# warmshao/ChatTTSPlus

Hardware: AMD Instinct MI355X
Metric: decode tokens/s (higher is better)
Workload: dtype f32

## Files before the change

chatttsplus_amd/csrc/gpt_engine.hip:

```cpp
#include <fcntl.h>
#include <stdarg.h>
#include <stdio.h>
#include <stdlib.h>
#include <string.h>
#include <sys/file.h>
#include <sys/stat.h>
#include <unistd.h>

#include <cmath>
#include <map>
#include <mutex>
#include <string>
#include <atomic>
#include <thread>
#include <vector>

#include "../../include/ctts_hip.h"
#include "kernels.h"
#include "persist.h"
#include "roctx_range.h"

static thread_local char g_err[512] = "";
void ctts_set_error(const char* fmt, ...) {
    va_list ap;
// ... 44 lines not shown
    float* logits_text = nullptr;
    float* lnf = nullptr;
    float* emb_code = nullptr;
    float* emb_text = nullptr;
    int vocab_text = 0;
    int vocab_text_head = 0;
    float* rope = nullptr;
    float *rope_pre = nullptr, *rope_dec = nullptr;
    int rope_n = 0;
    char* kv = nullptr;
    size_t kv_bytes = 0;
    float* sk_scratch = nullptr; size_t sk_cap_floats = 0;
    float *x_dec = nullptr, *x_last = nullptr, *x_pre = nullptr, *q_buf = nullptr, *part_ml = nullptr, *part_o = nullptr, *logits = nullptr;
    void* act = nullptr;
    void* attn_packed = nullptr;
    void* norm_packed = nullptr;
    int split_rows = 4;
    float* dpart = nullptr;
    int launched = 0;
    int nbg2_rows = 33;
    int force_splits = 0;
    int down_sk_rows = 9;
    float* sk_slab = nullptr; int* sk_cnt = nullptr;
    int opt_gen = 0;
    int graph_gen = 0;
    int valu_rows = 2;
    int persist_rows = 0;
    bool persist_ok = false;
    char* pimg = nullptr;
    char* pimg_head = nullptr;
    int persist_delay_u = -1;
    int prefill_pp_blocks = 1;
    int prefill_small_blocks = 192;
    int prefill_ring4_blocks = 256;
    int prefill_sk_rows = 2048;
    int attn_wide_blocks = 0;
    int persist_share_keys = 384;
    int persist_lora = 1;
    int persist_heads = 1;
    unsigned long long* pl_g = nullptr;
    unsigned* pl_epoch = nullptr;
    int* pl_error = nullptr;
    unsigned long long* pl_ts = nullptr;
    int pl_ts_on = 0;
    int persist_fault = 0;
    int persist_pair_keys = 704;
// ... 212 lines not shown
    {"persistent_share_keys", &ctts_gpt::persist_share_keys, 64, 384, OPT_MAX, OPT_MAX, OPT_RW, 0, HOOK_NONE},
    {"persistent_lora", &ctts_gpt::persist_lora, OPT_ANY, OPT_RW | OPT_FLAG, 0, HOOK_NONE},
    {"persistent_heads", &ctts_gpt::persist_heads, OPT_ANY, OPT_RW | OPT_FLAG, 0, HOOK_NONE},
    {"persistent_layers_per_launch", &ctts_gpt::persist_lpl, OPT_MIN(0), OPT_RW, 0, HOOK_NONE},
    {"persistent_schedule", &ctts_gpt::persist_sched, 1, 1, 3, 1, OPT_RW, 0, HOOK_NONE},
    {"lora_fold", &ctts_gpt::lora_fold, 0, 1, 3, 1, OPT_RW, 0, HOOK_NONE},
    {"persistent_fault", &ctts_gpt::persist_fault, OPT_MIN(0), OPT_RW, 0, HOOK_NONE},
    {"persistent_pair_keys", &ctts_gpt::persist_pair_keys, OPT_MIN(0), OPT_RW, 0, HOOK_NONE},
    {"persistent_max_keys", &ctts_gpt::persist_max_keys, OPT_MIN(0), OPT_RW, 0, HOOK_NONE},
    {"persistent_splits", &ctts_gpt::persist_splits, OPT_RANGE(0, PL_SMAX), OPT_RW, 0, HOOK_NONE},
    {"persistent_pace", &ctts_gpt::persist_pace, 0, -1, 64, 64, OPT_RW, 0, HOOK_NONE},
    {"persistent_delay_att", &ctts_gpt::persist_delay_att, OPT_RANGE(0, 256), OPT_RW, 0, HOOK_NONE},
    {"persistent_delay", &ctts_gpt::persist_delay, OPT_RANGE(0, 256), OPT_RW, 0, HOOK_NONE},
    {"persistent_delay_act", &ctts_gpt::persist_delay_act, OPT_RANGE(0, 256), OPT_RW, 0, HOOK_NONE},
    {"persistent_delay_x", &ctts_gpt::persist_delay_x, OPT_RANGE(0, 256), OPT_RW, 0, HOOK_NONE},
    {"persistent_nap_qkv", &ctts_gpt::persist_nap_qkv, OPT_RANGE(0, 256), OPT_RW, 0, HOOK_NONE},
    {"persistent_nap", &ctts_gpt::persist_nap, OPT_RANGE(0, 256), OPT_RW, 0, HOOK_NONE},
    {"persistent_poll", &ctts_gpt::persist_poll, OPT_ANY, OPT_RW, 0, HOOK_POLL},
    {"persistent_timestamps", &ctts_gpt::pl_ts_on, OPT_ANY, OPT_RW | OPT_FLAG, 0, HOOK_TIMESTAMPS},
    {"decode_splits", &ctts_gpt::force_splits, OPT_ANY, OPT_RW | OPT_PIN, 1, HOOK_DECODE_SPLITS},
    {"split_rows", &ctts_gpt::split_rows, OPT_RANGE(0, 32), OPT_RW | OPT_PIN, 0, HOOK_NONE},
    {"nbg2_rows", &ctts_gpt::nbg2_rows, OPT_MIN(17), OPT_RW | OPT_PIN, 0, HOOK_NONE},
    {"down_splitk_rows", &ctts_gpt::down_sk_rows, OPT_MIN(0), OPT_RW | OPT_PIN, 1, HOOK_NONE},
    {"graph_steps", &ctts_gpt::graph_steps, OPT_RANGE(1, 64), OPT_RW, 0, HOOK_NONE},
    {"graph_steps_persistent", &ctts_gpt::graph_steps_persist, OPT_RANGE(1, 64), OPT_RW, 0, HOOK_NONE},
    {"text_rows_live", &ctts_gpt::text_live, OPT_ANY, OPT_R, 0, HOOK_NONE},
    {"lora_mlp_live", &ctts_gpt::lora_mlp, OPT_ANY, OPT_R, 0, HOOK_NONE},
};
static const OptRow* find_option(const char* name, int access) {
    for (const OptRow& o : g_options) if (!strcmp(name, o.name)) return (o.flags & access) ? &o : nullptr;
    return nullptr;
}

extern "C" int ctts_gpt_get_option(ctts_gpt* h, const char* name, int* value) {
    if (!h || !name || !value) { ctts_set_error("get_option: null argument"); return 1; }
    const OptRow* o = find_option(name, OPT_R);
    if (!o) { ctts_set_error("get_option: unknown option '%s'", name); return 1; }
    if (h->batch_inv && (o->flags & OPT_PIN)) *value = o->pin;
    else if (o->hook == HOOK_PERSIST_ROWS) *value = (h->persist_ok || !h->finalized) ? h->persist_rows : 0;
    else *value = h->*o->field;
    return 0;
}

extern "C" int ctts_gpt_set_option(ctts_gpt* h, const char* name, int value) {
    if (!h || !name) { ctts_set_error("set_option: null argument"); return 1; }
    const OptRow* o = find_option(name, OPT_W);
// ... 507 lines not shown
    {
        long cap = (long)MB * h->cfg.max_seq;
        cap = (cap + 255) / 256 * 256;
        h->pass_rows = (int)(cap < PASS_ROWS_MAX ? cap : PASS_ROWS_MAX);
        if (const char* pr = getenv("CTTS_PASS_ROWS")) { const int v = atoi(pr); if (v >= 256 && v < h->pass_rows) h->pass_rows = v / 256 * 256; }
    }
    const int PASS_ROWS = h->pass_rows;
    const size_t act_bytes = (size_t)((PASS_ROWS + PASS_PAD) / 16) * (h->I / (h->esz == 2 ? 32 : 16)) * 1024;
    if (dev_alloc(h, (void**)&h->x_dec, (size_t)CTTS_MAX_B * H * 4) || dev_alloc(h, (void**)&h->x_last, (size_t)CTTS_MAX_B * H * 4) ||
        dev_alloc(h, (void**)&h->x_pre, (size_t)PASS_ROWS * H * 4) ||
        dev_alloc(h, (void**)&h->q_buf, (size_t)PASS_ROWS * H * 4) ||
        dev_alloc(h, (void**)&h->part_ml, (size_t)(CTTS_MAX_B + 32) * NH * SMAX * 2 * 4) ||
        dev_alloc(h, (void**)&h->part_o, (size_t)(CTTS_MAX_B + 32) * NH * SMAX * CTTS_HEAD_DIM * 4) ||
        dev_alloc(h, (void**)&h->logits, (size_t)CTTS_MAX_B * (h->NVQ * h->V > h->vocab_text_head ? h->NVQ * h->V : h->vocab_text_head) * 4) || dev_alloc(h, &h->act, act_bytes) || dev_alloc(h, (void**)&h->rope_pre, (size_t)MB * h->cfg.max_seq * 64 * 4) ||
        dev_alloc(h, (void**)&h->rope_dec, (size_t)CTTS_MAX_B * 64 * 4) || dev_alloc(h, (void**)&h->dpart, (size_t)32 * 4 * H * 4) || dev_alloc(h, &h->attn_packed, (size_t)((PASS_ROWS + PASS_PAD) / 16) * (H / (h->esz == 2 ? 32 : 16)) * 1024) ||
        dev_alloc(h, &h->norm_packed, (size_t)((PASS_ROWS + PASS_PAD) / 16) * (H / (h->esz == 2 ? 32 : 16)) * 1024) ||
        dev_alloc(h, (void**)&h->meta_pre, (size_t)MB * h->cfg.max_seq * sizeof(RowMeta)) ||
        dev_alloc(h, (void**)&h->meta_dec, CTTS_MAX_B * sizeof(RowMeta)) || dev_alloc(h, (void**)&h->meta_dec0, CTTS_MAX_B * sizeof(RowMeta)) ||
        dev_alloc(h, (void**)&h->st, sizeof(DevState)) || dev_alloc(h, (void**)&h->last_rows, CTTS_MAX_B * 4) ||
        dev_alloc(h, (void**)&h->dyn, sizeof(SamplerDyn)) || dev_alloc(h, (void**)&h->hist_ring, (size_t)CTTS_MAX_B * CTTS_NUM_VQ * 16 * 4) ||
        dev_alloc(h, (void**)&h->finend, (size_t)CTTS_MAX_B * (sizeof(RowState) + sizeof(RowSampling))) || dev_alloc(h, (void**)&h->sat, 4) ||
        dev_alloc(h, (void**)&h->cknobs, (size_t)CTTS_MAX_B * sizeof(RowSampling)) ||
        dev_alloc(h, (void**)&h->sk_slab, (size_t)(H / 16) * (CTTS_MAX_B / 16) * 4 * 256 * 4) || dev_alloc(h, (void**)&h->sk_cnt, (size_t)(H / 16) * (CTTS_MAX_B / 16) * 4) ||
        dev_alloc(h, (void**)&h->cx, (size_t)CTTS_MAX_B * H * 4) || dev_alloc(h, (void**)&h->crope, (size_t)CTTS_MAX_B * 64 * 4) ||
        dev_alloc(h, (void**)&h->cmeta, CTTS_MAX_B * sizeof(RowMeta)) || dev_alloc(h, (void**)&h->cring, (size_t)CTTS_MAX_B * CTTS_NUM_VQ * 16 * 4) ||
        dev_alloc(h, (void**)&h->cfin, (size_t)CTTS_MAX_B * sizeof(RowState)) || dev_alloc(h, (void**)&h->keep_dev, CTTS_MAX_B * 4) ||
        dev_alloc(h, &h->xh, (size_t)((CTTS_MAX_B + 32) / 16) * (H / (h->esz == 2 ? 32 : 16)) * 1024) || dev_alloc(h, (void**)&h->ssq, (size_t)(CTTS_MAX_B + 32) * (H / 16) * 4) ||
        dev_alloc(h, (void**)&h->scale_o, (size_t)(CTTS_MAX_B + 32) * 4) || dev_alloc(h, (void**)&h->scale_d, (size_t)(CTTS_MAX_B + 32) * 4) ||
        dev_alloc(h, (void**)&h->rope_dec0, (size_t)CTTS_MAX_B * 64 * 4))
        return 1;
    if (h->wsplit) {
        const size_t rows = (size_t)PASS_ROWS + PASS_PAD;
        if (dev_alloc(h, &h->sp_x_hi, rows * H * 2) || dev_alloc(h, &h->sp_x_lo, rows * H * 2) || dev_alloc(h, &h->sp_act_hi, rows * h->I * 2) || dev_alloc(h, &h->sp_act_lo, rows * h->I * 2)) return 1;
        h->sk_cap_floats = (size_t)4 * (size_t)(((PASS_ROWS < 2048 ? PASS_ROWS : 2048) + 127) / 128 * 128) * H;
        if (dev_alloc(h, (void**)&h->sk_scratch, h->sk_cap_floats * 4)) return 1;
    }
    h->knobs = (RowSampling*)(h->finend + CTTS_MAX_B);
    CTTS_HIP_CHECK(hipHostMalloc((void**)&h->host_pin, 64));
    {
        auto it = h->host.find("emb_text.weight");
        if (it != h->host.end() && it->second.size() % H == 0) {
            h->vocab_text = (int)(it->second.size() / H);
            if (dev_alloc(h, (void**)&h->emb_text, it->second.size() * 4)) return 1;
            CTTS_HIP_CHECK(hipMemcpy(h->emb_text, it->second.data(), it->second.size() * 4, hipMemcpyHostToDevice));
        }
    }
// ... 47 lines not shown
static inline int decode_splits(const ctts_gpt* h, int B, int L) {
    const int forced = tuning(h).force_splits;
    if (h->lora_rows) return 1;
    if (forced) return forced;
    int cap = 256 / (B * h->NH);
    cap = cap < 1 ? 1 : (cap > SMAX ? SMAX : cap);
    if (B <= 2) return cap;
    if (B >= 8) return 1;
    const int want = (L + 767) / 768;
    return want < 1 ? 1 : (want > cap ? cap : want);
}

struct StreamForm { bool parts, xh, logits, split; int nbg, valu; };
static inline int decode_nbg(const Tuning& t, int R, bool split) { return (R <= 16 || R < (split ? t.split_nbg2_rows : t.nbg2_rows)) ? 1 : 2; }
static StreamForm stream_form(const ctts_gpt* h, bool parts, bool xh, bool logits, bool split) {
    const Tuning t = tuning(h);
    return {parts, xh, logits, split, decode_nbg(t, h->B, split), (h->cfg.dtype == CTTS_DTYPE_F32 && h->B <= t.valu_rows) ? 1 : 0};
}
static inline StreamForm plain_form(const ctts_gpt* h) { return stream_form(h, false, false, false, false); }

struct LayerPlan {
    bool lora, lmlp;
    int S, nbg, chunks, dts, pf_kb, valu, wide_blocks, anchor, prefill_sk_rows;
    bool splitd, prepack, pfg, pfs, xhm, spd, down_sk, fuse_heads;
    int persist, per, pace, poll, delay_act, delay_u;
    StreamForm form;
};
static LayerPlan plan_layers(const ctts_gpt* h, int R, bool decode, DecodePath path) {
    LayerPlan p = {};
    const Tuning t = tuning(h);
    const int dt = h->cfg.dtype;
    p.S = path.splits; p.lora = h->lora_rows != 0; p.lmlp = p.lora && h->lora_mlp != 0;
    const bool spd_ok = decode && dt == CTTS_DTYPE_F32 && h->xh_mode && h->split_ok && h->wsplit != nullptr && !p.lora && p.S == 1 &&
                        t.split_dec_rows > 0 && R >= t.split_dec_rows && R > t.split_rows;
    p.nbg = decode ? decode_nbg(t, R, spd_ok) : (R <= 16 ? 1 : 2);
    p.chunks = (R + 16 * p.nbg - 1) / (16 * p.nbg);
    p.splitd = decode && (R <= t.split_rows) && (p.nbg == 1) && !p.lora;
    p.prepack = !decode && (p.nbg == 2) && (R > 64) && !h->no_prepack;
    p.pfg = p.prepack && (dt == CTTS_DTYPE_F16) && h->prefill_gemm_rows > 0 && (R >= h->prefill_gemm_rows) && !p.lora;
    p.pfs = (dt == CTTS_DTYPE_F32) && h->wsplit != nullptr &&
            (t.inv ? (!decode && h->split_ok) : (p.prepack && h->split_rows_min > 0 && (R >= h->split_rows_min)));
    p.xhm = decode && h->xh_mode && !p.splitd;
    p.spd = p.xhm && spd_ok;
    p.dts = p.spd ? 2 : dt;
    p.pf_kb = (p.xhm && !p.lora && (p.spd || (dt == CTTS_DTYPE_F16 && R >= 17))) ? h->prefetch_kb : 0;
    p.valu = (decode && dt == CTTS_DTYPE_F32 && R <= t.valu_rows && !p.lora) ? 1 : 0;
    p.down_sk = (p.nbg == 1 || p.spd) && R >= t.down_sk_rows && t.down_sk_rows > 0;
    p.wide_blocks = t.attn_wide_blocks; p.anchor = t.inv ? 1 : 0; p.prefill_sk_rows = t.prefill_sk_rows;
    p.form = stream_form(h, p.splitd, p.xhm, false, p.spd);
    p.persist = (decode && h->pimg != nullptr && R <= PL_MAXR) ? path.persist : 0;
    if (p.persist) {
        p.fuse_heads = h->persist_heads && R <= 2 && !h->text_mode && h->text_live == 0 && h->persist_sched == 3 && h->pimg_head != nullptr && h->dyn != nullptr;
        p.form = stream_form(h, false, false, p.fuse_heads, false);
        p.per = (h->persist_lpl > 0 && h->persist_lpl < h->L) ? h->persist_lpl : h->L;
        p.pace = h->persist_pace < 0 ? (R <= 2 ? 3 : 2) : h->persist_pace; p.poll = (h->persist_poll < 0) ? 0 : h->persist_poll;
        p.delay_act = h->persist_delay_act + 2 * (R - 1); p.delay_u = h->persist_delay_u < 0 ? 14 + 2 * R : h->persist_delay_u;
    }
    return p;
}

static int run_layers(ctts_gpt* h, float* x, const RowMeta* meta, const float* rope_rows, int R, DecodePath path, const DevState* st, hipStream_t s, StreamForm* form = nullptr) {
    const LayerPlan p = plan_layers(h, R, st != nullptr, path);
    const int dt = h->cfg.dtype, S = p.S, nbg = p.nbg, NB = 16 * nbg, chunks = p.chunks, dts = p.dts;
    const bool lora = p.lora, lmlp = p.lmlp, splitd = p.splitd, prepack = p.prepack, pfg = p.pfg, pfs = p.pfs, xhm = p.xhm, spd = p.spd;
    if (form) *form = p.form;
    if (p.persist) {
        for (int l = 0; l < h->L; l += p.per) {
            PersistArgs pa = {};
            if (p.fuse_heads && l + p.per >= h->L) {
                pa.heads = 1; pa.hw = h->pimg_head; pa.logits = h->logits; pa.n_valid = h->NVQ * h->V; pa.lnf = h->lnf; pa.dyn = h->dyn; pa.rows = h->finend;
// ... 111 lines not shown
            if (launch_gemm(dts, nbg, PRO_XH, EPI_SWIGLU, g3, chunks, s)) return 1;
        } else if (launch_gemm(dt, nbg, PRO_NORM, EPI_SWIGLU, g3, chunks, s)) return 1;
        GemmArgs g4 = a;
        g4.W = h->lw[l].d; g4.n_row_tiles = h->H / 16; g4.K = h->I; g4.xpacked = h->act; g4.x_out = x;
        if (lmlp) {
            if (pfs ? launch_lora_delta_down_split(h->sp_act_hi, h->sp_act_lo, meta, h->lora_slot_of_seq, h->lora_mA_d + mlp_l * 16 * h->I, h->lora_mB_d + mlp_l * 16 * h->H,
                                                   h->lora_mscale + mlp_l * 4, h->lora_do, R, h->H, h->I, s)
                    : launch_lora_delta_down(dt, h->act, nbg, meta, h->lora_slot_of_seq, h->lora_mA_d + mlp_l * 16 * h->I, h->lora_mB_d + mlp_l * 16 * h->H,
                                             h->lora_mscale + mlp_l * 4, h->lora_do, R, h->H, h->I, s)) return 1;
            g4.lora_delta = h->lora_do;
        }
        if (pfs) {
            if (launch_prefill_split_gemm(EPI_RESID, g4, h->lw[l].d_sp, h->sp_act_hi, h->sp_act_lo, nullptr, nullptr, sp_scale * 16.0f, sp_pol, s)) return 1;
        } else if (pfg) {
            if (launch_prefill_gemm(EPI_RESID, g4, s)) return 1;
        } else if (splitd) {
            g4.part_out = h->dpart; g4.ktiles_total = h->I / (h->esz == 2 ? 32 : 16);
            if (launch_gemm(dt, nbg, PRO_PACKED, EPI_PART, g4, chunks, s)) return 1;
        } else if (xhm) {
            g4.xh = h->xh; g4.ssq = h->ssq; g4.scale_in = h->scale_d;
            if (spd) g4.W = h->lw[l].d_sp;
            if (p.down_sk) {
                g4.ktiles_total = h->I / ((h->esz == 2 || spd) ? 32 : 16); g4.sk_slab = h->sk_slab; g4.sk_cnt = h->sk_cnt;
                if (launch_gemm(dts, nbg, PRO_PACKED, EPI_RESID_XH_SK, g4, chunks, s)) return 1;
            } else if (launch_gemm(dts, nbg, PRO_PACKED, EPI_RESID_XH, g4, chunks, s)) return 1;
        } else if (launch_gemm(dt, nbg, PRO_PACKED, EPI_RESID, g4, chunks, s)) return 1;
    }
    return 0;
}
static int run_heads(ctts_gpt* h, bool write_hidden, StreamForm form, hipStream_t s, bool mixed_text = false) {
    const int nbg = form.nbg, chunks = (h->B + 16 * nbg - 1) / (16 * nbg);
    const bool text = h->text_mode || mixed_text;
    GemmArgs a = {};
    a.st = h->st; a.R = h->B; a.eps = 1e-6f; a.meta = h->meta_dec;
    a.valu = form.valu;
    const int nv = text ? h->vocab_text_head : h->NVQ * h->V;
    a.W = text ? h->whead_text : h->whead; a.n_row_tiles = (nv + 15) / 16; a.K = h->H; a.x = h->x_dec; a.lnw = h->lnf;
    a.logits = mixed_text ? h->logits_text : h->logits; a.n_valid = nv;
    a.dyn = (write_hidden && !mixed_text) ? h->dyn : nullptr;
    a.rows = h->finend;
    a.opart = h->dpart; a.np = form.parts ? 4 : 0;
    if (form.xh && !text && h->xh_heads && (!form.split || h->whead_sp != nullptr)) {
        a.xh = h->xh; a.ssq = h->ssq; a.scale_in = h->scale_d;
        if (form.split) a.W = h->whead_sp;
        return launch_gemm(form.split ? 2 : h->cfg.dtype, nbg, PRO_XH, EPI_LOGITS, a, chunks, s);
    }
// ... 7 lines not shown
        if (!h->text_rows_on || !h->dyn_text || !h->logits_text) {
            ctts_set_error("sample / decode: a row of the batch is a text row (mode 1) but ctts_gpt_enable_text_rows has not been called for this generate state");
            return 1;
        }
        StreamForm tf = form;
        tf.logits = false;
        if (run_heads(h, false, tf, s, true)) return 1;
    }
    SamplerArgs sa = {};
    sa.dyn = h->dyn; sa.logits = h->logits; sa.V = h->text_mode ? h->vocab_text_head : h->V; sa.B = h->B; sa.st = h->st;
    sa.text_mode = h->text_mode; sa.mixed = mixed ? 1 : 0;
    sa.emb_code = h->text_mode ? h->emb_text : h->emb_code; sa.H = h->H; sa.x_next = h->x_dec; sa.meta = h->meta_dec; sa.rope = h->rope; sa.rope_rows = h->rope_dec;
    sa.hist_ring = h->hist_ring; sa.finend = h->finend;
    if (launch_sampler(sa, h->B, s)) return 1;
    if (!mixed) return 0;
    sa.dyn = h->dyn_text; sa.logits = h->logits_text; sa.V = h->vocab_text_head; sa.text_mode = 1; sa.emb_code = h->emb_text;
    return launch_sampler(sa, h->B, s);
}

static int reset_state(ctts_gpt* h, bool keep_draw, hipStream_t s) {
    h->launched = 0;
    CTTS_HIP_CHECK(hipMemsetAsync(&h->st->step, 0, 4, s));
    if (!keep_draw) CTTS_HIP_CHECK(hipMemsetAsync(&h->st->draw, 0, 4, s));
    CTTS_HIP_CHECK(hipMemsetAsync(&h->st->all_done, 0, 8, s));
    CTTS_HIP_CHECK(hipMemcpyAsync(h->meta_dec, h->meta_dec0, h->B * sizeof(RowMeta), hipMemcpyDeviceToDevice, s));
    CTTS_HIP_CHECK(hipMemsetAsync(h->io.finish, 0, h->B * 4, s));
    CTTS_HIP_CHECK(hipMemsetAsync(h->io.end_idx, 0, h->B * 4, s));
    if (!keep_draw) {
        CTTS_HIP_CHECK(hipMemcpyAsync(h->finend, h->rows_host.data(), h->B * sizeof(RowState), hipMemcpyHostToDevice, s));
    } else {
        if (launch_restart_rows(h->finend, h->B, s)) return 1;
        h->row_ctx.assign(h->B, h->T);
    }
    CTTS_HIP_CHECK(hipMemsetAsync(h->hist_ring, 0xFF, (size_t)h->B * CTTS_NUM_VQ * 16 * 4, s));
    return 0;
}

static int seat_row_adapters(ctts_gpt* h, int B, const char* who, hipStream_t s) {
    if (h->lora_slot_host.empty()) return 0;
    if (h->lora_req_host.empty()) h->lora_slot_host.assign(CTTS_MAX_B, -1);
    else h->lora_slot_host = h->lora_req_host;
    bool any = false;
    for (int b = 0; b < CTTS_MAX_B; ++b) { h->lora_row_slots[b] = (signed char)h->lora_slot_host[b]; any = any || (b < B && h->lora_slot_host[b] >= 0); }
    h->lora_rows = any ? 1 : 0;
    h->lora_mlp = 0;
    for (int b = 0; b < B; ++b) if (lora_slot_has_mlp(h, h->lora_slot_host[b])) h->lora_mlp = 1;
// ... 520 lines not shown
    (void)advance_rows(h, n_steps);
    h->launched += n_steps;
    bool persistent = false;
    for (const auto& sg : h->segs) persistent = persistent || sg.path.persist != 0;
    PersistTurnGuard turn(persistent, s);
    if (turn.rc) { ctts_set_error("decode: hipStreamWaitEvent failed"); return 1; }
    for (const auto& sg : h->segs) if (run_segment(h, sg, use_graph != 0, true, s)) return 1;
    return 0;
}

extern "C" int ctts_gpt_progress(ctts_gpt* h, int32_t* steps_done, int32_t* all_finished, void* stream) {
    if (!h) { ctts_set_error("null handle"); return 1; }
    hipStream_t s = (hipStream_t)stream;
    CTTS_HIP_CHECK(hipMemcpyAsync(h->host_pin, h->st, 16, hipMemcpyDeviceToHost, s));
    h->host_pin[12] = 0;
    if (h->pl_error) CTTS_HIP_CHECK(hipMemcpyAsync(h->host_pin + 12, h->pl_error, 4, hipMemcpyDeviceToHost, s));
    CTTS_HIP_CHECK(hipStreamSynchronize(s));
    if (steps_done) *steps_done = h->host_pin[0];
    if (all_finished) *all_finished = h->host_pin[2];
    if (h->host_pin[12] == 7) {
        ctts_set_error("per-utterance LoRA: a projection tile gave up waiting for its low-rank term (lora_worker.h); use options={'lora_fold': 0}");
        return 1;
    }
    if (h->host_pin[12] != 0) {
        ctts_set_error("persistent decode layer: a workgroup gave up waiting on edge %d (2 = q|k|v -> attention, 3 = attention -> o_proj, 4 = o_proj -> gate|up, "
                       "5 = gate|up -> down); is the GPU shared with another process?  Use options={'persistent_rows': 0}", h->host_pin[12]);
        return 1;
    }
    return 0;
}

extern "C" int ctts_gpt_progress_enqueue(ctts_gpt* h, int32_t* host_pinned4, void* stream) {
    if (!h || !host_pinned4) { ctts_set_error("progress_enqueue: null argument"); return 1; }
    CTTS_HIP_CHECK(hipMemcpyAsync(host_pinned4, h->st, 16, hipMemcpyDeviceToHost, (hipStream_t)stream));
    return 0;
}

extern "C" int ctts_gpt_saturations(ctts_gpt* h, int32_t* count, void* stream) {
    if (!h || !count || !h->sat) { ctts_set_error("saturations: bad argument"); return 1; }
    CTTS_HIP_CHECK(hipMemcpyAsync(h->host_pin + 8, h->sat, 4, hipMemcpyDeviceToHost, (hipStream_t)stream));
    CTTS_HIP_CHECK(hipStreamSynchronize((hipStream_t)stream));
    *count = h->host_pin[8];
    return 0;
}

extern "C" int ctts_gpt_rows_enqueue(ctts_gpt* h, int32_t* host_pinned_2B, void* stream) {
// ... 316 lines not shown
```

chatttsplus_amd/csrc/kernels.h:

```cpp
#pragma once
#include "common.h"

enum { PRO_NORM = 0, PRO_ATTN = 1, PRO_PACKED = 2, PRO_NORM_P = 3, PRO_XH = 4 };
enum { EPI_QKV = 0, EPI_RESID = 1, EPI_SWIGLU = 2, EPI_LOGITS = 3, EPI_RESID_P = 4, EPI_PART = 5, EPI_RESID_XH = 6, EPI_RESID_XH_SK = 7 };
#define CTTS_NPART 4

typedef unsigned long long lora_u64;
struct LoraFold {
    const float* A;
    const float* B;
    const float* scale;
    const float* lnw;
    signed char slots[CTTS_MAX_B];
    signed char ranks[32];
    lora_u64* g;
    lora_u64* g_o;
    int* err;
    int layer;
    int diag;
};

struct WPrefetch {
    const void* ptr;
    unsigned unit_bytes;
    unsigned n_units;
};

// ... 18 lines not shown
    const void* xpacked;
    float* x_out;
    float* q_out;
    void* k_cache;
    void* v_cache;
    int Lmax;
    const RowMeta* meta;
    const float* rope_rows;
    void* act_out;
    float* logits;
    int n_valid;
    void* xh;
    float* ssq;
    const float* scale_in;
    float* scale_out;
    const float* lora_delta;
    int lora_gu;
    LoraFold lf;
    int lora_w;
    int* sat;
    const RowState* rows;
    float* sk_slab;
    int* sk_cnt;
    WPrefetch pf;
    int pf_blocks;
    int valu;
};

struct AttnArgs {
    const float* q;
    const void* k_cache;
    const void* v_cache;
    int Lmax;
    int NH;
    int R;
    int S;
    const RowMeta* meta;
    const DevState* st;
    float* part_ml;
    float* part_o;
    void* packed_out;
    int nbg;
    int packed_split;
    int T, row0;
    int wide_blocks;
    int anchor;
// ... 152 lines not shown
```

chatttsplus_amd/csrc/skinny_gemm.hip:

```cpp
#include "kernels.h"
#include "lora_worker.h"

#define ATT_SMAX 8

template <typename WT> struct Mma;
template <> struct Mma<half_t> {
    __device__ static inline f32x4 run(half8 a, half8 b, f32x4 c) {
        return __builtin_amdgcn_mfma_f32_16x16x32_f16(a, b, c, 0, 0, 0);
    }
};
template <> struct Mma<float> {
    __device__ static inline f32x4 run(f32x4 a, f32x4 b, f32x4 c) {
        c = __builtin_amdgcn_mfma_f32_16x16x4f32(a[0], b[0], c, 0, 0, 0);
        c = __builtin_amdgcn_mfma_f32_16x16x4f32(a[1], b[1], c, 0, 0, 0);
        c = __builtin_amdgcn_mfma_f32_16x16x4f32(a[2], b[2], c, 0, 0, 0);
        c = __builtin_amdgcn_mfma_f32_16x16x4f32(a[3], b[3], c, 0, 0, 0);
        return c;
    }
};

struct SplitFrag { half8 hi, lo; };
template <> struct Mma<split_t> {
    __device__ static inline f32x4 run(const SplitFrag& a, const SplitFrag& b, f32x4 c) {
        c = __builtin_amdgcn_mfma_f32_16x16x32_f16(a.lo, b.hi, c, 0, 0, 0);
        c = __builtin_amdgcn_mfma_f32_16x16x32_f16(a.hi, b.lo, c, 0, 0, 0);
        c = __builtin_amdgcn_mfma_f32_16x16x32_f16(a.hi, b.hi, c, 0, 0, 0);
// ... 68 lines not shown
        const char* p = (const char*)pf.ptr + (size_t)u * pf.unit_bytes + (unsigned)(tid * 16);
        for (unsigned off = 0; off < pf.unit_bytes; off += WAVES * 1024)
            __builtin_amdgcn_global_load_lds((gptr_t)(p + off), (lptr_t)dst, 16, 0, 0);
    }
}

template <typename WT, int NBG, int WAVES, int KPW, int PRO, int EPI, int RT = 1, int VR = 0, bool LORA = false>
__global__ __launch_bounds__(WAVES * 64) void skinny_gemm_kernel(const int* done_p, const void* Wq, const void* in0, const void* in1,
                                                                  const float* resid_in, const int R, const int misc, const GemmArgs a) {
    static_assert(RT == 1 || EPI == EPI_QKV || EPI == EPI_SWIGLU, "multi-tile blocks: QKV / SwiGLU epilogues only");
    static_assert(VR == 0 || (sizeof(WT) == 4 && NBG == 1 && RT == 1 && PRO != PRO_XH && VR <= 4), "VALU products: fp32, one 16-row chunk, <= 4 rows");
    constexpr bool VALU = VR > 0;
    constexpr bool SPLIT = (WTraits<WT>::TILE_BYTES == 2048);
    typedef typename FragOf<WT>::type frag;
    constexpr int KT = WTraits<WT>::KT;
    constexpr int KTILES = WAVES * KPW;
    constexpr int K = KTILES * KT;
    constexpr int NB = 16 * NBG;
    constexpr int XS_BYTES = (PRO == PRO_PACKED || PRO == PRO_XH) ? 0 : NBG * KTILES * WTraits<WT>::TILE_BYTES;
    constexpr int PER = K / 256;
    extern __shared__ __attribute__((aligned(16))) char smem[];

    int done_v = 0;
    if (done_p != nullptr) done_v = vload_flag(done_p);
#define CTTS_EXIT_IF_DONE() if (__builtin_amdgcn_readfirstlane(done_v)) return

    const int tid = threadIdx.x, lane = tid & 63, wave = tid >> 6;
    constexpr bool PFCAP = (EPI == EPI_RESID_XH) && (PRO == PRO_PACKED) && (K == 768) && VR == 0 && !LORA;
    if constexpr (PFCAP) {
        const int xreal = (int)((unsigned)misc >> 22);
        if (__builtin_expect(xreal != 0 && (int)blockIdx.x >= xreal, 0)) {
            if (blockIdx.y == 0 && blockIdx.z == 0) {
                weight_prefetch<WAVES>(a.pf, (int)blockIdx.x - xreal, (int)gridDim.x - xreal, (int)blockIdx.x & 7, smem, tid);
            }
            return;
        }
    }
    const int chunk = blockIdx.y;
    const int row0 = chunk * NB;
    constexpr bool LORA_QKV = LORA && (EPI == EPI_QKV) && (K == 768) && (VR == 0) && (PRO == PRO_NORM || PRO == PRO_XH);
    constexpr bool LORA_O = LORA && (EPI == EPI_RESID || EPI == EPI_RESID_XH) && (K == 768) && (VR == 0) && (PRO == PRO_PACKED);
    constexpr bool LORA_GU = LORA && (EPI == EPI_SWIGLU) && (VR == 0);
    static_assert(!LORA || LORA_QKV || LORA_O || LORA_GU, "LoRA: the q/k/v and o_proj launches of a decode step (workers), the gate|up launch (epilogue term)");
    const int lw = (LORA_QKV || LORA_O) ? ((misc >> 15) & 0x7F) : 0;
    int lora_draw = 0;
#define CTTS_LORA_TAG_LO ((unsigned)a.lf.layer * 2u + (LORA_O ? 1u : 0u))
// ... 214 lines not shown
    }

    constexpr bool PREB = !VALU && (PRO == PRO_PACKED) && ((RT == 1 && NBG * KPW * (SPLIT ? 2 : 1) <= 12) || NBG * KPW * (SPLIT ? 2 : 1) <= 6);
    frag bpre[NBG][KPW];
    f32x4 bv[(VALU && PRO == PRO_PACKED) ? VR : 1][KPW];
    if (PRO == PRO_PACKED) {
        if (VALU) {
            const f32x4* xq = (const f32x4*)in0 + (size_t)chunk * NBG * kt_all * 64 + (lane & 48);
#pragma unroll
            for (int n = 0; n < VR; ++n)
#pragma unroll
                for (int i = 0; i < KPW; ++i) bv[n][i] = xq[(size_t)(kt_off + wave * KPW + i) * 64 + n];
        }
        if (PREB) {
#pragma unroll
            for (int g = 0; g < NBG; ++g)
#pragma unroll
                for (int i = 0; i < KPW; ++i) bpre[g][i] = FragIO<WT>::load(in0, (size_t)chunk * NBG * kt_all + (size_t)(g * kt_all + kt_off + wave * KPW + i), lane);
        }
        CTTS_ISSUE_WEIGHT_LOADS();
        CTTS_EXIT_IF_DONE();
    }
    float* fac_s = (float*)(smem + XS_BYTES + WAVES * NBG * 1024);
    if (PRO == PRO_XH) {
        constexpr int LPR = 64 / NB, PPL = 48 / LPR;
        f32x4 sq[PPL / 4];
        float sc_in = 1.f;
        const int n_f = lane / LPR, part = lane % LPR;
        const bool frow = (wave == WAVES - 1) && (row0 + n_f < R);
        if (frow) {
            const f32x4* sp = (const f32x4*)((const float*)in1 + (size_t)(row0 + n_f) * 48 + part * PPL);
#pragma unroll
            for (int i = 0; i < PPL / 4; ++i) sq[i] = sp[i];
            sc_in = resid_in[row0 + n_f];
        }
        {
#pragma unroll
            for (int g = 0; g < NBG; ++g)
#pragma unroll
                for (int i = 0; i < KPW; ++i) bpre[g][i] = FragIO<WT>::load(in0, (size_t)chunk * NBG * KTILES + (size_t)(g * KTILES + wave * KPW + i), lane);
        }
        CTTS_ISSUE_WEIGHT_LOADS();
        CTTS_EXIT_IF_DONE();
        if (wave == WAVES - 1) {
            float ss = 0.f;
            if (frow) {
#pragma unroll
                for (int i = 0; i < PPL / 4; ++i) ss += (sq[i][0] + sq[i][1]) + (sq[i][2] + sq[i][3]);
            }
            ss += dpp_f<DPP_XOR1>(ss);
            if (LPR == 4) ss += dpp_f<DPP_XOR2>(ss);
            if (frow && part == 0) {
                const float rs = 1.0f / sqrtf(ss / (float)K + a.eps);
                fac_s[n_f] = SPLIT ? rs / (sc_in * CTTS_SPLIT_WSCALE) : rs / sc_in;
                if (EPI == EPI_LOGITS) fac_s[NB + n_f] = rs;
                if (rt0 == 0 && a.scale_out != nullptr)
                    a.scale_out[row0 + n_f] = __builtin_bit_cast(float, __builtin_bit_cast(unsigned, rs) & 0x7F800000u);
            }
        }
    }

    float accv[VALU ? VR : 1];
    if constexpr (VALU) {
#pragma unroll
        for (int n = 0; n < VR; ++n) accv[n] = 0.f;
#pragma unroll
// ... 39 lines not shown
#pragma unroll
    for (int i = 0; i < LPEEK; ++i) lpeek[i] = 0;
    const bool ltake = (LORA_QKV || LORA_O) && lw != 0 && a.lf.diag != 2;
    if constexpr (LORA_QKV) {
        if (ltake && tid < 8 * NB && row0 + (tid >> 3) < R) {
#pragma unroll
            for (int ti = 0; ti < RT; ++ti) {
                const int rt = rt0 + ti, which = rt / (K / 16), within = rt % (K / 16);
                const lora_u64* gp = a.lf.g + ((size_t)(row0 + (tid >> 3)) * 3 + which) * K + (within >> 2) * CTTS_HEAD_DIM + ((within & 3) << 3) + (tid & 7);
                lpeek[2 * ti] = lora_peek(gp); lpeek[2 * ti + 1] = lora_peek(gp + 32);
            }
        }
    }
    if constexpr (LORA_O) {
        if (ltake) {
#pragma unroll
            for (int u = 0; u < RITEMS; ++u) {
                const int t = tid + u * WAVES * 64, r = row0 + (t >> 4);
                if (t < 16 * NB && r < R) lpeek[u] = lora_peek(a.lf.g_o + (size_t)r * 768 + rt0 * 16 + (t & 15));
            }
        }
    }

    float* red = (float*)(smem + XS_BYTES);
#pragma unroll
    for (int ti = 0; ti < RT; ++ti) {
    const int rt = rt0 + ti;
    if (ti > 0) __syncthreads();
    if constexpr (VALU) {
        if (lane < 16) {
#pragma unroll
            for (int n = 0; n < VR; ++n) red[(wave * VR + n) * 16 + lane] = accv[n];
        }
    } else {
#pragma unroll
        for (int g = 0; g < NBG; ++g) *(f32x4*)(red + ((wave * NBG + g) * 64 + lane) * 4) = acc[ti][g];
    }
    __syncthreads();
    auto c_elem = [&](int i, int n) -> float {
        if constexpr (VALU) {
            if (n >= VR) return 0.f;
            float sum = 0.f;
#pragma unroll
            for (int w = 0; w < WAVES; ++w) sum += red[(w * VR + n) * 16 + i];
            return sum;
        }
        const float* q = red + (((n >> 4) * 64) + ((i >> 2) << 4) + (n & 15)) * 4 + (i & 3);
        float sum = 0.f;
#pragma unroll
        for (int w = 0; w < WAVES; ++w) sum += q[w * NBG * 256];
        if (PRO == PRO_XH) sum *= fac_s[n];
        else if (SPLIT) sum *= ((K == 3072 || SLICED) ? CTTS_SPLIT_ACT_SCALE : 1.0f) / CTTS_SPLIT_WSCALE;
        return sum;
    };

    float sk_v[RITEMS];
    if constexpr (EPI == EPI_RESID_XH_SK) {
        static_assert(RT == 1, "split-K combine: one weight row tile per block");
        constexpr int SLAB = 256 * NBG;
        const int nz = gridDim.z, slice = blockIdx.z;
        float* const slab0 = a.sk_slab + ((size_t)(rt * gridDim.y + chunk) * nz) * SLAB;
        int* const lastp = (int*)(red + WAVES * NBG * 256);
#pragma unroll
        for (int u = 0; u < RITEMS; ++u) {
            const int t = tid + u * WAVES * 64;
            sk_v[u] = 0.f;
            if (t < SLAB) {
                sk_v[u] = c_elem(t & 15, t >> 4);
                __hip_atomic_store(slab0 + (size_t)slice * SLAB + t, sk_v[u], __ATOMIC_RELAXED, __HIP_MEMORY_SCOPE_AGENT);
            }
        }
        asm volatile("s_waitcnt vmcnt(0)" ::: "memory");
        __syncthreads();
        if (tid == 0) {
            int* const cnt = a.sk_cnt + rt * gridDim.y + chunk;
            const int ticket = __hip_atomic_fetch_add(cnt, 1, __ATOMIC_RELAXED, __HIP_MEMORY_SCOPE_AGENT);
            if (ticket == nz - 1) __hip_atomic_store(cnt, 0, __ATOMIC_RELAXED, __HIP_MEMORY_SCOPE_AGENT);
            *lastp = (ticket == nz - 1) ? 1 : 0;
        }
        __syncthreads();
        if (*lastp == 0) return;
#pragma unroll
        for (int u = 0; u < RITEMS; ++u) {
            const int t = tid + u * WAVES * 64;
            if (t < SLAB) {
                float pq[4];
#pragma unroll
                for (int q = 0; q < 4; ++q)
                    pq[q] = (q >= nz) ? 0.f : (q == slice) ? sk_v[u] : __hip_atomic_load(slab0 + (size_t)q * SLAB + t, __ATOMIC_RELAXED, __HIP_MEMORY_SCOPE_AGENT);
                sk_v[u] = ((pq[0] + pq[1]) + pq[2]) + pq[3];
            }
        }
    }
    if (EPI == EPI_RESID || EPI == EPI_RESID_P || EPI == EPI_LOGITS || EPI == EPI_PART || EPI == EPI_RESID_XH || EPI == EPI_RESID_XH_SK) {
#pragma unroll
        for (int u = 0; u < RITEMS; ++u) {
            const int t = tid + u * WAVES * 64;
            if (t >= 16 * NB) continue;
            const int n = t >> 4, i = t & 15;
            const int r = row0 + n;
            if (r >= R) continue;
            const int col = rt * 16 + i;
            float v = (EPI == EPI_RESID_XH_SK) ? sk_v[u] : c_elem(i, n);
            if ((EPI == EPI_RESID || EPI == EPI_RESID_P || EPI == EPI_RESID_XH || EPI == EPI_RESID_XH_SK) && a.lora_delta != nullptr)
                v += a.lora_delta[(size_t)r * (a.n_row_tiles * 16) + col];
            if constexpr (LORA_O) {
                if (ltake) v += lora_take_peeked(lpeek[u], a.lf.g_o + (size_t)r * 768 + col, lora_tag_of(lora_draw, CTTS_LORA_TAG_LO), a.lf.err);
            }
            if (EPI == EPI_PART) {
                a.part_out[((size_t)r * gridDim.z + blockIdx.z) * (a.n_row_tiles * 16) + col] = v;
            } else if (EPI == EPI_RESID || EPI == EPI_RESID_P) {
                const float xn = resid_pf[u] + v;
                a.x_out[(size_t)r * (a.n_row_tiles * 16) + col] = xn;
            } else if (EPI == EPI_RESID_XH || EPI == EPI_RESID_XH_SK) {
// ... 42 lines not shown
                        d0 = __builtin_bit_cast(float, (unsigned)lpeek[2 * ti]); d1 = __builtin_bit_cast(float, (unsigned)lpeek[2 * ti + 1]);
                    } else lora_take2(gp, gp + 32, tg, a.lf.err, d0, d1);
                    ya += d0; yb += d1;
                }
            }
            const float va2 = ya, vb2 = yb;
            if (which < 2) {
                ya = __fadd_rn(__fmul_rn(va2, rope_c[ti]), __fmul_rn(-vb2, rope_s[ti]));
                yb = __fadd_rn(__fmul_rn(vb2, rope_c[ti]), __fmul_rn(va2, rope_s[ti]));
            }
            if (which == 0) {
                float* q = a.q_out + ((size_t)r * NH + h) * CTTS_HEAD_DIM;
                q[d] = ya; q[d + 32] = yb;
            } else {
                typedef typename WTraits<WT>::cache_t CT;
                CT* c = (CT*)(which == 1 ? a.k_cache : a.v_cache) +
                        (((size_t)meta_pf.seq * NH + h) * a.Lmax + meta_pf.slot) * CTTS_HEAD_DIM;
                c[d] = (CT)ya; c[d + 32] = (CT)yb;
            }
        }
    }
    }
    if (PRO == PRO_XH && EPI == EPI_LOGITS) {
        float* const hid_out = (a.dyn != nullptr) ? ((SamplerDynPtr)a.dyn)->hidden_out : nullptr;
        if (hid_out != nullptr && rt0 == 0) {
            const int rows = min(NB, R - row0);
            for (int n = wave; n < rows; n += WAVES) {
                const int r = row0 + n;
                const float rs = fac_s[NB + n];
                const f32x4* xr = (const f32x4*)(a.x + (size_t)r * K);
                const int4 rstate = *(const int4*)(a.rows + r);
                if (rstate.x != 0) continue;
                float* hrow = hid_out + (size_t)a.rows[r].out * ((SamplerDynPtr)a.dyn)->hidden_stride + (size_t)rstate.y * K;
#pragma unroll
                for (int i = 0; i < PER; ++i) {
                    const int k = 4 * (lane + 64 * i);
                    const f32x4 v = xr[lane + 64 * i], w = *(const f32x4*)(a.lnw + k);
                    *(f32x4*)(hrow + k) = (f32x4){w[0] * (v[0] * rs), w[1] * (v[1] * rs), w[2] * (v[2] * rs), w[3] * (v[3] * rs)};
                }
            }
        }
    }
}

template <typename WT, int NBG, int WAVES, int KPW, int PRO, int EPI, int RT = 1, int VR = 0, bool LORA = false>
static int launch_one(const GemmArgs& a, int chunks, hipStream_t s, bool configure_only) {
    constexpr int KTILES = WAVES * KPW;
    constexpr int XS = (PRO == PRO_PACKED || PRO == PRO_XH) ? 0 : NBG * KTILES * WTraits<WT>::TILE_BYTES;
    constexpr bool LORA_OK = LORA && (KTILES * WTraits<WT>::KT == 768) && (VR == 0) &&
                             ((EPI == EPI_QKV && (PRO == PRO_NORM || PRO == PRO_XH)) || ((EPI == EPI_RESID || EPI == EPI_RESID_XH) && PRO == PRO_PACKED));
    constexpr int LDS0 = XS + WAVES * NBG * 1024 + 16 * 16 * NBG * 4 + 16;
    constexpr int LDS = (LORA_OK && LDS0 < 6272) ? 6272 : LDS0;
    auto kern = skinny_gemm_kernel<WT, NBG, WAVES, KPW, PRO, EPI, RT, VR, LORA>;
    if (configure_only) {
        CTTS_HIP_CHECK(hipFuncSetAttribute((const void*)kern, hipFuncAttributeMaxDynamicSharedMemorySize, LDS));
        return 0;
    }
    int nz = 1;
    if (EPI == EPI_PART || EPI == EPI_RESID_XH_SK) {
        if (a.ktiles_total % KTILES || a.K != a.ktiles_total * WTraits<WT>::KT) { ctts_set_error("skinny_gemm: split-K tiling mismatch"); return 1; }
        nz = a.ktiles_total / KTILES;
    } else if (a.K != KTILES * WTraits<WT>::KT) {
        ctts_set_error("skinny_gemm: K=%d does not match the compiled tiling %d", a.K, KTILES * WTraits<WT>::KT);
        return 1;
    }
    if (a.n_row_tiles % RT) { ctts_set_error("skinny_gemm: %d row tiles not a multiple of %d", a.n_row_tiles, RT); return 1; }
    const int* done_p = a.st ? &a.st->all_done : nullptr;
    const void* in0 = (PRO == PRO_ATTN) ? (const void*)a.part_ml : (PRO == PRO_PACKED) ? (const void*)a.xpacked : (PRO == PRO_XH) ? (const void*)a.xh : (const void*)a.x;
    const void* in1 = (PRO == PRO_ATTN) ? (const void*)a.part_o : (PRO == PRO_NORM_P) ? (const void*)a.opart : (PRO == PRO_XH) ? (const void*)a.ssq :
                      (EPI == EPI_RESID_XH || EPI == EPI_RESID_XH_SK) ? (const void*)a.scale_in : nullptr;
    if (EPI == EPI_RESID_XH_SK && (nz > 4 || a.sk_slab == nullptr || a.sk_cnt == nullptr)) { ctts_set_error("skinny_gemm: split-K combine needs <= 4 slices and its slabs"); return 1; }
    const float* resid_arg = (PRO == PRO_XH) ? a.scale_in : (const float*)a.x_out;
    if (a.lora_w != 0 && (!LORA_OK || a.lora_w != (EPI == EPI_QKV ? 3 : 1) * 16 * NBG || a.st == nullptr || a.ktiles_total > 255)) {
        ctts_set_error("skinny_gemm: this launch cannot carry LoRA workers (pro %d epi %d workers %d)", PRO, EPI, a.lora_w);
        return 1;
    }
    const int xreal = a.n_row_tiles / RT + a.lora_w;
    constexpr bool PFCAP = (EPI == EPI_RESID_XH) && (PRO == PRO_PACKED) && (KTILES * WTraits<WT>::KT == 768) && VR == 0 && !LORA;
    const bool pf_on = PFCAP && a.pf_blocks >= 8 && a.pf.ptr != nullptr && (a.pf.unit_bytes % (WAVES * 1024)) == 0 && xreal < 1024;
    const int npf = pf_on ? (a.pf_blocks & ~7) : 0;
    const int misc = (a.np & 0x7) | ((a.S & 0xF) << 3) | ((a.ktiles_total & 0xFF) << 7) | ((a.lora_w & 0x7F) << 15) | (int)((unsigned)(npf ? xreal : 0) << 22);
    hipLaunchKernelGGL(kern, dim3(xreal + npf, chunks, nz), dim3(WAVES * 64), LDS, s, done_p, a.W, in0, in1, resid_arg, a.R, misc, a);
    CTTS_HIP_CHECK(hipGetLastError());
    return 0;
}

#ifndef CTTS_RT_NORM
#define CTTS_RT_NORM 2
#endif
#ifndef CTTS_RT_XH
#define CTTS_RT_XH 1
#endif
template <typename WT, int NBG>
static int dispatch(int pro, int epi, const GemmArgs& a, int chunks, hipStream_t s, bool cfg) {
// ... 194 lines not shown
```

Baseline: 3909.

## Hand off split-K down-projection partials via tagged granules instead of slab counters

In decode, the split-K down projection now has non-final K slices publish each partial element together with a tag built from the draw and layer into a granule array. The final slice peeks these early and spins until the tags match, replacing the slab write, counter atomic and last-arriver combine. This removes a counter round-trip and fence from the critical path, at the cost of a spin-wait that can time out and report an error. Separately, the logits kernel's hidden-row output is now loaded early and written with one float4 per thread instead of a per-wave loop.

```diff
diff --git a/chatttsplus_amd/csrc/gpt_engine.hip b/chatttsplus_amd/csrc/gpt_engine.hip
--- a/chatttsplus_amd/csrc/gpt_engine.hip
+++ b/chatttsplus_amd/csrc/gpt_engine.hip
@@ -90,6 +90,8 @@
     int force_splits = 0;
     int down_sk_rows = 9;
     float* sk_slab = nullptr; int* sk_cnt = nullptr;
+    int down_granules = 1;
+    unsigned long long* sk_gran = nullptr;
     int opt_gen = 0;
     int graph_gen = 0;
     int valu_rows = 2;
@@ -348,6 +350,7 @@
     {"split_rows", &ctts_gpt::split_rows, OPT_RANGE(0, 32), OPT_RW | OPT_PIN, 0, HOOK_NONE},
     {"nbg2_rows", &ctts_gpt::nbg2_rows, OPT_MIN(17), OPT_RW | OPT_PIN, 0, HOOK_NONE},
     {"down_splitk_rows", &ctts_gpt::down_sk_rows, OPT_MIN(0), OPT_RW | OPT_PIN, 1, HOOK_NONE},
+    {"down_granules", &ctts_gpt::down_granules, OPT_ANY, OPT_RW | OPT_FLAG, 0, HOOK_NONE},
     {"graph_steps", &ctts_gpt::graph_steps, OPT_RANGE(1, 64), OPT_RW, 0, HOOK_NONE},
     {"graph_steps_persistent", &ctts_gpt::graph_steps_persist, OPT_RANGE(1, 64), OPT_RW, 0, HOOK_NONE},
     {"text_rows_live", &ctts_gpt::text_live, OPT_ANY, OPT_R, 0, HOOK_NONE},
@@ -901,6 +904,7 @@
         dev_alloc(h, (void**)&h->finend, (size_t)CTTS_MAX_B * (sizeof(RowState) + sizeof(RowSampling))) || dev_alloc(h, (void**)&h->sat, 4) ||
         dev_alloc(h, (void**)&h->cknobs, (size_t)CTTS_MAX_B * sizeof(RowSampling)) ||
         dev_alloc(h, (void**)&h->sk_slab, (size_t)(H / 16) * (CTTS_MAX_B / 16) * 4 * 256 * 4) || dev_alloc(h, (void**)&h->sk_cnt, (size_t)(H / 16) * (CTTS_MAX_B / 16) * 4) ||
+        dev_alloc(h, (void**)&h->sk_gran, CTTS_SK_GRANULES * 8) || (!h->pl_error && dev_alloc(h, (void**)&h->pl_error, 4)) ||
         dev_alloc(h, (void**)&h->cx, (size_t)CTTS_MAX_B * H * 4) || dev_alloc(h, (void**)&h->crope, (size_t)CTTS_MAX_B * 64 * 4) ||
         dev_alloc(h, (void**)&h->cmeta, CTTS_MAX_B * sizeof(RowMeta)) || dev_alloc(h, (void**)&h->cring, (size_t)CTTS_MAX_B * CTTS_NUM_VQ * 16 * 4) ||
         dev_alloc(h, (void**)&h->cfin, (size_t)CTTS_MAX_B * sizeof(RowState)) || dev_alloc(h, (void**)&h->keep_dev, CTTS_MAX_B * 4) ||
@@ -994,7 +998,7 @@
 struct LayerPlan {
     bool lora, lmlp;
     int S, nbg, chunks, dts, pf_kb, valu, wide_blocks, anchor, prefill_sk_rows;
-    bool splitd, prepack, pfg, pfs, xhm, spd, down_sk, fuse_heads;
+    bool splitd, prepack, pfg, pfs, xhm, spd, down_sk, down_gran, fuse_heads;
     int persist, per, pace, poll, delay_act, delay_u;
     StreamForm form;
 };
@@ -1018,6 +1022,7 @@
     p.pf_kb = (p.xhm && !p.lora && (p.spd || (dt == CTTS_DTYPE_F16 && R >= 17))) ? h->prefetch_kb : 0;
     p.valu = (decode && dt == CTTS_DTYPE_F32 && R <= t.valu_rows && !p.lora) ? 1 : 0;
     p.down_sk = (p.nbg == 1 || p.spd) && R >= t.down_sk_rows && t.down_sk_rows > 0;
+    p.down_gran = p.down_sk && decode && h->down_granules && h->sk_gran != nullptr && h->L <= 64 && h->H == 768 && R <= CTTS_MAX_B;
     p.wide_blocks = t.attn_wide_blocks; p.anchor = t.inv ? 1 : 0; p.prefill_sk_rows = t.prefill_sk_rows;
     p.form = stream_form(h, p.splitd, p.xhm, false, p.spd);
     p.persist = (decode && h->pimg != nullptr && R <= PL_MAXR) ? path.persist : 0;
@@ -1175,6 +1180,7 @@
             if (spd) g4.W = h->lw[l].d_sp;
             if (p.down_sk) {
                 g4.ktiles_total = h->I / ((h->esz == 2 || spd) ? 32 : 16); g4.sk_slab = h->sk_slab; g4.sk_cnt = h->sk_cnt;
+                if (p.down_gran) { g4.sk_gran = h->sk_gran; g4.sk_err = h->pl_error; g4.sk_layer = l; }
                 if (launch_gemm(dts, nbg, PRO_PACKED, EPI_RESID_XH_SK, g4, chunks, s)) return 1;
             } else if (launch_gemm(dts, nbg, PRO_PACKED, EPI_RESID_XH, g4, chunks, s)) return 1;
         } else if (launch_gemm(dt, nbg, PRO_PACKED, EPI_RESID, g4, chunks, s)) return 1;
@@ -1228,6 +1234,7 @@
     h->launched = 0;
     CTTS_HIP_CHECK(hipMemsetAsync(&h->st->step, 0, 4, s));
     if (!keep_draw) CTTS_HIP_CHECK(hipMemsetAsync(&h->st->draw, 0, 4, s));
+    if (!keep_draw && h->sk_gran) CTTS_HIP_CHECK(hipMemsetAsync(h->sk_gran, 0, CTTS_SK_GRANULES * 8, s));
     CTTS_HIP_CHECK(hipMemsetAsync(&h->st->all_done, 0, 8, s));
     CTTS_HIP_CHECK(hipMemcpyAsync(h->meta_dec, h->meta_dec0, h->B * sizeof(RowMeta), hipMemcpyDeviceToDevice, s));
     CTTS_HIP_CHECK(hipMemsetAsync(h->io.finish, 0, h->B * 4, s));
@@ -1794,6 +1801,10 @@
         ctts_set_error("per-utterance LoRA: a projection tile gave up waiting for its low-rank term (lora_worker.h); use options={'lora_fold': 0}");
         return 1;
     }
+    if (h->host_pin[12] == 8) {
+        ctts_set_error("decode: the down projection's combining workgroup gave up waiting for a K slice's partial tile (skinny_gemm.hip step 4b); use options={'down_granules': 0}");
+        return 1;
+    }
     if (h->host_pin[12] != 0) {
         ctts_set_error("persistent decode layer: a workgroup gave up waiting on edge %d (2 = q|k|v -> attention, 3 = attention -> o_proj, 4 = o_proj -> gate|up, "
                        "5 = gate|up -> down); is the GPU shared with another process?  Use options={'persistent_rows': 0}", h->host_pin[12]);
diff --git a/chatttsplus_amd/csrc/kernels.h b/chatttsplus_amd/csrc/kernels.h
--- a/chatttsplus_amd/csrc/kernels.h
+++ b/chatttsplus_amd/csrc/kernels.h
@@ -3,6 +3,7 @@
 
 enum { PRO_NORM = 0, PRO_ATTN = 1, PRO_PACKED = 2, PRO_NORM_P = 3, PRO_XH = 4 };
 enum { EPI_QKV = 0, EPI_RESID = 1, EPI_SWIGLU = 2, EPI_LOGITS = 3, EPI_RESID_P = 4, EPI_PART = 5, EPI_RESID_XH = 6, EPI_RESID_XH_SK = 7 };
+#define CTTS_SK_GRANULES ((size_t)(768 / 16) * (CTTS_MAX_B / 16) * 3 * 256)
 #define CTTS_NPART 4
 
 typedef unsigned long long lora_u64;
@@ -67,6 +68,9 @@
     const RowState* rows;
     float* sk_slab;
     int* sk_cnt;
+    lora_u64* sk_gran;
+    int* sk_err;
+    int sk_layer;
     WPrefetch pf;
     int pf_blocks;
     int valu;
diff --git a/chatttsplus_amd/csrc/skinny_gemm.hip b/chatttsplus_amd/csrc/skinny_gemm.hip
--- a/chatttsplus_amd/csrc/skinny_gemm.hip
+++ b/chatttsplus_amd/csrc/skinny_gemm.hip
@@ -2,6 +2,31 @@
 #include "lora_worker.h"
 
 #define ATT_SMAX 8
+
+#define SK_ERR_CODE 8
+__device__ inline unsigned sk_tag_of(int draw_v, int layer) { return ((unsigned)draw_v + 1u) * 64u + (unsigned)layer; }
+__device__ inline int4 vload_hdr(const int* p) {
+    int z;
+    asm volatile("v_mov_b32 %0, 0" : "=v"(z));
+    return ((const int4*)p)[z];
+}
+__device__ inline void sk_take_peeked(lora_u64 (&x)[3], const lora_u64* p, int stride, int n, unsigned tag, int* err) {
+    const lora_u64* const p1 = p + (n > 1 ? stride : 0);
+    const lora_u64* const p2 = p + (n > 2 ? 2 * (size_t)stride : 0);
+#pragma unroll 1
+    for (unsigned spins = 0; spins < LORA_SPIN_LIMIT; ++spins) {
+        if ((unsigned)(x[0] >> 32) == tag && (n < 2 || (unsigned)(x[1] >> 32) == tag) && (n < 3 || (unsigned)(x[2] >> 32) == tag)) return;
+        if (spins != 0) __builtin_amdgcn_s_sleep(1);
+        x[0] = __hip_atomic_load(p, __ATOMIC_RELAXED, __HIP_MEMORY_SCOPE_AGENT);
+        x[1] = __hip_atomic_load(p1, __ATOMIC_RELAXED, __HIP_MEMORY_SCOPE_AGENT);
+        x[2] = __hip_atomic_load(p2, __ATOMIC_RELAXED, __HIP_MEMORY_SCOPE_AGENT);
+    }
+    bool miss = false;
+#pragma unroll
+    for (int q = 0; q < 3; ++q)
+        if (q < n && (unsigned)(x[q] >> 32) != tag) { x[q] = 0; miss = true; }
+    if (miss && err != nullptr) atomicCAS(err, 0, SK_ERR_CODE);
+}
 
 template <typename WT> struct Mma;
 template <> struct Mma<half_t> {
@@ -116,6 +141,10 @@
     extern __shared__ __attribute__((aligned(16))) char smem[];
 
     int done_v = 0;
+    int sk_draw = 0;
+    if constexpr (EPI == EPI_RESID_XH_SK) {
+        if (done_p != nullptr) { const int4 hdr = vload_hdr(done_p - 2); done_v = hdr.z; sk_draw = hdr.y; }
+    } else
     if (done_p != nullptr) done_v = vload_flag(done_p);
 #define CTTS_EXIT_IF_DONE() if (__builtin_amdgcn_readfirstlane(done_v)) return
 
@@ -376,6 +405,9 @@
         CTTS_EXIT_IF_DONE();
     }
     float* fac_s = (float*)(smem + XS_BYTES + WAVES * NBG * 1024);
+    f32x4 h_x = {0.f, 0.f, 0.f, 0.f}, h_w = {0.f, 0.f, 0.f, 0.f};
+    float* h_base = nullptr;
+    int h_stride = 0, h_fin = 1, h_end = 0, h_out = 0;
     if (PRO == PRO_XH) {
         constexpr int LPR = 64 / NB, PPL = 48 / LPR;
         f32x4 sq[PPL / 4];
@@ -396,6 +428,17 @@
         }
         CTTS_ISSUE_WEIGHT_LOADS();
         CTTS_EXIT_IF_DONE();
+        if constexpr (EPI == EPI_LOGITS) {
+            static_assert(K / 4 <= WAVES * 64, "hidden row: one float4 per thread");
+            asm volatile("" : "=v"(h_x), "=v"(h_w), "=v"(h_fin), "=v"(h_end), "=v"(h_out));
+            if (a.dyn != nullptr && rt0 < NB && row0 + rt0 < R) {
+                const int r = row0 + rt0;
+                h_base = ((SamplerDynPtr)a.dyn)->hidden_out; h_stride = ((SamplerDynPtr)a.dyn)->hidden_stride;
+                const int4 s0 = *(const int4*)(a.rows + r), s1 = *((const int4*)(a.rows + r) + 1);
+                h_fin = s0.x; h_end = s0.y; h_out = s1.z;
+                if (tid < K / 4) { h_x = ((const f32x4*)(a.x + (size_t)r * K))[tid]; h_w = ((const f32x4*)a.lnw)[tid]; }
+            }
+        }
         if (wave == WAVES - 1) {
             float ss = 0.f;
             if (frow) {
@@ -481,6 +524,25 @@
         }
     }
 
+    constexpr int SKP = (EPI == EPI_RESID_XH_SK) ? RITEMS : 1;
+    lora_u64 skpeek[SKP][3];
+    bool sk_gran = false;
+    if constexpr (EPI == EPI_RESID_XH_SK) {
+        sk_gran = a.sk_gran != nullptr;
+        const int nprod = (int)gridDim.z - 1;
+#pragma unroll
+        for (int u = 0; u < SKP; ++u) {
+            asm volatile("" : "=v"(skpeek[u][0]), "=v"(skpeek[u][1]), "=v"(skpeek[u][2]));
+            const int t = tid + u * WAVES * 64;
+            if (sk_gran && nprod > 0 && (int)blockIdx.z == nprod && t < 16 * NB && row0 + (t >> 4) < R) {
+                const lora_u64* gp = a.sk_gran + ((size_t)(rt0 * gridDim.y + chunk) * 3) * (256 * NBG) + t;
+                skpeek[u][0] = lora_peek(gp);
+                skpeek[u][1] = lora_peek(gp + (nprod > 1 ? 256 * NBG : 0));
+                skpeek[u][2] = lora_peek(gp + (nprod > 2 ? 2 * 256 * NBG : 0));
+            }
+        }
+    }
+
     float* red = (float*)(smem + XS_BYTES);
 #pragma unroll
     for (int ti = 0; ti < RT; ++ti) {
@@ -520,6 +582,34 @@
         const int nz = gridDim.z, slice = blockIdx.z;
         float* const slab0 = a.sk_slab + ((size_t)(rt * gridDim.y + chunk) * nz) * SLAB;
         int* const lastp = (int*)(red + WAVES * NBG * 256);
+        if (__builtin_expect(sk_gran, 1)) {
+            lora_u64* const g0 = a.sk_gran + ((size_t)(rt * gridDim.y + chunk) * 3) * SLAB;
+            asm volatile("" : "+v"(sk_draw));
+            const unsigned tag = sk_tag_of(sk_draw, a.sk_layer);
+            if (slice < nz - 1) {
+#pragma unroll
+                for (int u = 0; u < RITEMS; ++u) {
+                    const int t = tid + u * WAVES * 64;
+                    if (t < SLAB && row0 + (t >> 4) < R) lora_publish(g0 + (size_t)slice * SLAB + t, tag, c_elem(t & 15, t >> 4));
+                }
+                return;
+            }
+#pragma unroll
+            for (int u = 0; u < RITEMS; ++u) {
+                const int t = tid + u * WAVES * 64;
+                sk_v[u] = 0.f;
+                if (t < SLAB && row0 + (t >> 4) < R) {
+                    const float own = c_elem(t & 15, t >> 4);
+                    if (nz > 1) sk_take_peeked(skpeek[u], g0 + t, SLAB, nz - 1, tag, a.sk_err);
+                    float pq[4];
+#pragma unroll
+                    for (int q = 0; q < 3; ++q)
+                        pq[q] = (q >= nz) ? 0.f : (q == nz - 1) ? own : __builtin_bit_cast(float, (unsigned)skpeek[u][q]);
+                    pq[3] = (nz == 4) ? own : 0.f;
+                    sk_v[u] = ((pq[0] + pq[1]) + pq[2]) + pq[3];
+                }
+            }
+        } else {
 #pragma unroll
         for (int u = 0; u < RITEMS; ++u) {
             const int t = tid + u * WAVES * 64;
@@ -549,6 +639,7 @@
                     pq[q] = (q >= nz) ? 0.f : (q == slice) ? sk_v[u] : __hip_atomic_load(slab0 + (size_t)q * SLAB + t, __ATOMIC_RELAXED, __HIP_MEMORY_SCOPE_AGENT);
                 sk_v[u] = ((pq[0] + pq[1]) + pq[2]) + pq[3];
             }
+        }
         }
     }
     if (EPI == EPI_RESID || EPI == EPI_RESID_P || EPI == EPI_LOGITS || EPI == EPI_PART || EPI == EPI_RESID_XH || EPI == EPI_RESID_XH_SK) {
@@ -637,23 +728,11 @@
     }
     }
     if (PRO == PRO_XH && EPI == EPI_LOGITS) {
-        float* const hid_out = (a.dyn != nullptr) ? ((SamplerDynPtr)a.dyn)->hidden_out : nullptr;
-        if (hid_out != nullptr && rt0 == 0) {
-            const int rows = min(NB, R - row0);
-            for (int n = wave; n < rows; n += WAVES) {
-                const int r = row0 + n;
-                const float rs = fac_s[NB + n];
-                const f32x4* xr = (const f32x4*)(a.x + (size_t)r * K);
-                const int4 rstate = *(const int4*)(a.rows + r);
-                if (rstate.x != 0) continue;
-                float* hrow = hid_out + (size_t)a.rows[r].out * ((SamplerDynPtr)a.dyn)->hidden_stride + (size_t)rstate.y * K;
-#pragma unroll
-                for (int i = 0; i < PER; ++i) {
-                    const int k = 4 * (lane + 64 * i);
-                    const f32x4 v = xr[lane + 64 * i], w = *(const f32x4*)(a.lnw + k);
-                    *(f32x4*)(hrow + k) = (f32x4){w[0] * (v[0] * rs), w[1] * (v[1] * rs), w[2] * (v[2] * rs), w[3] * (v[3] * rs)};
-                }
-            }
+        asm volatile("" : "+v"(h_x), "+v"(h_w), "+v"(h_fin), "+v"(h_end), "+v"(h_out));
+        if (h_base != nullptr && h_fin == 0 && tid < K / 4) {
+            const float rs = fac_s[NB + rt0];
+            float* hrow = h_base + (size_t)h_out * h_stride + (size_t)h_end * K;
+            ((f32x4*)hrow)[tid] = (f32x4){h_w[0] * (h_x[0] * rs), h_w[1] * (h_x[1] * rs), h_w[2] * (h_x[2] * rs), h_w[3] * (h_x[3] * rs)};
         }
     }
 }
@@ -684,7 +763,14 @@
     const void* in0 = (PRO == PRO_ATTN) ? (const void*)a.part_ml : (PRO == PRO_PACKED) ? (const void*)a.xpacked : (PRO == PRO_XH) ? (const void*)a.xh : (const void*)a.x;
     const void* in1 = (PRO == PRO_ATTN) ? (const void*)a.part_o : (PRO == PRO_NORM_P) ? (const void*)a.opart : (PRO == PRO_XH) ? (const void*)a.ssq :
                       (EPI == EPI_RESID_XH || EPI == EPI_RESID_XH_SK) ? (const void*)a.scale_in : nullptr;
+    if (EPI == EPI_RESID_XH_SK && a.sk_gran != nullptr) {
+        if (nz > 4 || a.st == nullptr || a.sk_layer < 0 || a.sk_layer > 63 || (size_t)a.n_row_tiles * chunks * 3 * 256 * NBG > CTTS_SK_GRANULES) {
+            ctts_set_error("skinny_gemm: split-K granule hand-off needs <= 4 slices, a decode step, a layer index 0..63 and %d x %d tiles within its granule array", a.n_row_tiles, chunks);
+            return 1;
+        }
+    } else
     if (EPI == EPI_RESID_XH_SK && (nz > 4 || a.sk_slab == nullptr || a.sk_cnt == nullptr)) { ctts_set_error("skinny_gemm: split-K combine needs <= 4 slices and its slabs"); return 1; }
+    if (PRO == PRO_XH && EPI == EPI_LOGITS && a.dyn != nullptr && a.n_row_tiles < 16 * NBG) { ctts_set_error("skinny_gemm: the heads' hidden rows need one row tile per row of a chunk"); return 1; }
     const float* resid_arg = (PRO == PRO_XH) ? a.scale_in : (const float*)a.x_out;
     if (a.lora_w != 0 && (!LORA_OK || a.lora_w != (EPI == EPI_QKV ? 3 : 1) * 16 * NBG || a.st == nullptr || a.ktiles_total > 255)) {
         ctts_set_error("skinny_gemm: this launch cannot carry LoRA workers (pro %d epi %d workers %d)", PRO, EPI, a.lora_w);
```

Result: no change. 3912, median of 2 (+0.1%).
